# rasmusbarr/nudge

Hardware: AMD Instinct MI355X
Metric: simulation steps/s (contacts solved/s alongside), 1M-box drop scene (higher is better)
Workload: dtype f32

## Files before the change

### nudge_amd/csrc/nh_solve.hip

```cpp
#include "nh_internal.h"
#include <type_traits>
#include <atomic>
#include <string.h>
#include "nh_solver.h"
#include "nh_narrowphase.h"

__global__ __launch_bounds__(256) void k_gravity(const nh_DevState* __restrict__ st, const uint32_t* __restrict__ active, nh_BodyMomentum* __restrict__ momentum,
                                                 float gx_dt, float gy_dt, float gz_dt, float damping) {
	uint32_t n = st->active;
	for (uint32_t k = blockIdx.x * blockDim.x + threadIdx.x; k < n; k += gridDim.x * blockDim.x) {
		uint32_t i = active[k];
		nh_BodyMomentum m = momentum[i];
		nh_gravity_damping(m.velocity, m.angular_velocity, gx_dt, gy_dt, gz_dt, damping);
		momentum[i] = m;
	}
}

__global__ __launch_bounds__(256) void k_advance(const nh_DevState* __restrict__ st, const uint32_t* __restrict__ active, nh_Transform* __restrict__ xf,
                                                 const nh_BodyMomentum* __restrict__ momentum, uint8_t* __restrict__ idle, float time_step) {
	uint32_t n = st->active;
	for (uint32_t k = blockIdx.x * blockDim.x + threadIdx.x; k < n; k += gridDim.x * blockDim.x) {
		uint32_t i = active[k];
		nh_Transform t = xf[i];
		nh_BodyMomentum m = momentum[i];
// ... 309 lines not shown
			for (int q = 0; q < M; ++q) cid[q] = (uint32_t)q < cnt ? adj[b + q] : 0u;
#pragma unroll
			for (int q = 0; q < M; ++q) {
				miss[q] = false; wx[q] = wy[q] = wz[q] = 0.0f;
				if ((uint32_t)q < cnt) {
					const uint32_t c = cid[q];
					is_a[q] = bodies[c].a == x;
					ctc[q] = contacts[c];
					if (FUSED) {
						const uint64_t t = cv.tags[c]; const uint32_t f = cv.features[c];
						const bool in = c < m;
						const uint64_t ct = in ? cv.ctags[c] : 0ull; const uint32_t cf = in ? cv.cfeatures[c] : 0u;
						nh_CachedContactImpulse wc = { { 0.0f, 0.0f, 0.0f }, 0.0f };
						if (in) wc = cv.cdata[c];
						const bool hit = in && ct == t && cf == f;
						if (hit) { wx[q] = wc.impulse[0]; wy[q] = wc.impulse[1]; wz[q] = wc.impulse[2]; }
						miss[q] = !hit;
					} else {
						float4 sv = states[c];
						s[q].normal = sv.x; s[q].friction_x = sv.y; s[q].friction_y = sv.z;
					}
				}
			}
			if (FUSED) {
#pragma unroll
				for (int q = 0; q < M; ++q) {
					if (miss[q]) {
						const uint32_t c = cid[q];
						const uint64_t t = cv.tags[c]; const uint32_t f = cv.features[c];
						uint32_t lo = 0, hi = m;
						while (lo < hi) { uint32_t mid = (lo + hi) >> 1; if (tag_less(cv.ctags[mid], cv.cfeatures[mid], t, f)) lo = mid + 1; else hi = mid; }
						if (lo < m && cv.ctags[lo] == t && cv.cfeatures[lo] == f) { nh_CachedContactImpulse w = cv.cdata[lo]; wx[q] = w.impulse[0]; wy[q] = w.impulse[1]; wz[q] = w.impulse[2]; }
					}
				}
			}
#pragma unroll
			for (int q = 0; q < M; ++q) {
				if ((uint32_t)q < cnt) {
					const nh_Contact& ct = ctc[q];
					nh_contact_in ci = { ct.position[0], ct.position[1], ct.position[2], ct.penetration, ct.normal[0], ct.normal[1], ct.normal[2], ct.friction };
					if (is_a[q]) nh_build_row(ci, posx, pos0, IX, I0, v.mass_inverse, z.mass_inverse, r[q]);
					else         nh_build_row(ci, pos0, posx, I0, IX, z.mass_inverse, v.mass_inverse, r[q]);
					if (FUSED) {
						if (is_a[q]) nh_warm_start(r[q], wx[q], wy[q], wz[q], v, z, s[q]);
						else         nh_warm_start(r[q], wx[q], wy[q], wz[q], z, v, s[q]);
					}
				}
			}
			for (uint32_t it = 0; it < iterations; ++it) {
#pragma unroll
				for (int q = 0; q < M; ++q) {
					if ((uint32_t)q < cnt) {
						if (is_a[q]) nh_apply_one(r[q], s[q], v, z); else nh_apply_one(r[q], s[q], z, v);
					}
				}
			}
#pragma unroll
			for (int q = 0; q < M; ++q)
				if ((uint32_t)q < cnt) {
					states[cid[q]] = make_float4(s[q].normal, s[q].friction_x, s[q].friction_y, 0.0f);
					nh_CachedContactImpulse o;
					nh_export_impulse(r[q], s[q], o.impulse[0], o.impulse[1], o.impulse[2]);
					o.unused = 0.0f;
					impulses[cid[q]] = o;
				}
		} else {
			const nh_inertia IXn = body_inertia(xf, props, x);
			const nh_Transform txn = xf[x];
			const nh_f3 posxn = nh_make3(txn.position[0], txn.position[1], txn.position[2]);
			for (uint32_t it = 0; it < iterations; ++it) {
				for (uint32_t q = b; q < e; ++q) {
					uint32_t c = adj[q];
					const bool x_is_a = bodies[c].a == x;
					nh_Contact ct = contacts[c];
					nh_contact_in ci = { ct.position[0], ct.position[1], ct.position[2], ct.penetration, ct.normal[0], ct.normal[1], ct.normal[2], ct.friction };
					nh_row r;
					if (x_is_a) nh_build_row(ci, posxn, pos0, IXn, I0, v.mass_inverse, z.mass_inverse, r);
					else        nh_build_row(ci, pos0, posxn, I0, IXn, z.mass_inverse, v.mass_inverse, r);
					float4 sv = states[c];
					nh_state s = { sv.x, sv.y, sv.z };
					if (x_is_a) nh_apply_one(r, s, v, z); else nh_apply_one(r, s, z, v);
					states[c] = make_float4(s.normal, s.friction_x, s.friction_y, 0.0f);
					if (it + 1 == iterations) {
						nh_CachedContactImpulse o;
						nh_export_impulse(r, s, o.impulse[0], o.impulse[1], o.impulse[2]);
						o.unused = 0.0f;
						impulses[c] = o;
					}
				}
			}
		}
		store_vel(momentum, x, v);
	}
}

#define NH_HINT_NONE 0xFFFFFFFFu

__device__ __forceinline__ bool cache_probe(const nh_CacheView& cv, uint32_t m, uint32_t guess, uint64_t t, uint32_t f, float& wx, float& wy, float& wz) {
	if (guess < m) {
		const uint64_t ct = cv.ctags[guess];
		const uint32_t cf = cv.cfeatures[guess];
		const float4 w = *reinterpret_cast<const float4*>(cv.cdata + guess);
		if (ct == t && cf == f) { wx = w.x; wy = w.y; wz = w.z; return true; }
	}
	return false;
}

__device__ __noinline__ float4 cache_search(const uint64_t* __restrict__ ctags, const uint32_t* __restrict__ cfeatures, const nh_CachedContactImpulse* __restrict__ cdata,
                                            uint32_t m, uint32_t guess, uint64_t t, uint32_t f) {
	const float4 none = make_float4(0.0f, 0.0f, 0.0f, 0.0f);
	uint32_t lo = 0, hi = m;
	if (guess != NH_HINT_NONE && m) {
		const uint32_t g = guess < m ? guess : m - 1;
		const uint32_t w0 = g >= 4 ? g - 4 : 0, w1 = g + 4 < m ? g + 4 : m;
		bool below = false, above = false;
		for (uint32_t k = w0; k < w1; ++k) {
			const uint64_t ct = ctags[k]; const uint32_t cf = cfeatures[k];
			if (ct == t && cf == f) return *reinterpret_cast<const float4*>(cdata + k);
			if (tag_less(ct, cf, t, f)) below = true; else above = true;
		}
		if ((below || w0 == 0) && (above || w1 == m)) return none;
		if (!below) hi = w0; else lo = w1;
	}
	while (lo < hi) { uint32_t mid = (lo + hi) >> 1; if (tag_less(ctags[mid], cfeatures[mid], t, f)) lo = mid + 1; else hi = mid; }
	if (lo < m && ctags[lo] == t && cfeatures[lo] == f) return *reinterpret_cast<const float4*>(cdata + lo);
	return none;
}

struct nh_ob_slot { float4 c0, c1, w; };

#ifndef NH_SOLVER_WPE
#define NH_SOLVER_WPE 2
#endif
struct nh_StillView { const uint32_t* body_rec; const uint32_t* body_pos; const uint32_t* cnt_sorted; uint32_t* start_sorted; const uint32_t* raw_feature; uint32_t* sc_feat; uint32_t* sc_count; uint32_t pair_cap;
                     const int2* delta; uint32_t parity; };

template<int MAXC, bool FUSED, bool CONTIG = false, int NW = 4, bool STILL = false, bool AHEAD = false, bool PAIR = false, bool PART = false>
__global__ __launch_bounds__(64 * NW) __attribute__((amdgpu_waves_per_eu(MAXC == 4 ? NH_SOLVER_WPE : 1, MAXC == 4 ? NH_SOLVER_WPE : 1))) void k_solve_one_body(uint32_t nbodies, const uint8_t* __restrict__ body_class, const uint32_t* __restrict__ off, const uint32_t* __restrict__ adj,
                                                        const nh_BodyPair* __restrict__ bodies, const nh_BodyProperties* __restrict__ props, nh_BodyMomentum* __restrict__ momentum,
                                                        float4* __restrict__ states, uint32_t iterations,
                                                        const nh_Contact* __restrict__ contacts, nh_Transform* xf, nh_CachedContactImpulse* __restrict__ impulses,
                                                        nh_CacheView cv, uint32_t* __restrict__ hint, uint32_t cls_a, uint32_t cls_b, uint32_t require_inert,
                                                        const uint2* __restrict__ simple = nullptr, nh_FusedStep fs = nh_FusedStep(), nh_StillView sv = nh_StillView(),
                                                        nh_AheadView av = nh_AheadView()) {
	constexpr int M = MAXC;
	const bool keep_states = !(require_inert & 2u);
	if (nbodies == 0u) return;
	if (STILL && CONTIG && NW == 1 && !PART && (fs.bits & 8u) && blockIdx.x != 0u) {
		const uint32_t x0 = blockIdx.x * 64u + threadIdx.x;
		const uint32_t i0 = (x0 < nbodies) ? (uint32_t)fs.idle[x0] : 0xffu;
		if (__builtin_amdgcn_ballot_w64(i0 != 0xffu) == 0ull) return;
	}
	uint32_t inert_word = (require_inert & 1u) ? cv.st->static_inert : 1u;
	if (STILL) {
		const nh_BodyMomentum m0 = momentum[0];
		const nh_BodyProperties p0 = props[0];
		const bool inert = nh_is_inert(m0.velocity, m0.angular_velocity, p0.inertia_inverse, p0.mass_inverse);
		if (!inert && blockIdx.x == 0 && threadIdx.x == 0) atomicMax(&const_cast<nh_DevState*>(cv.st)->still_failed_seq, fs.seq);
		if (!inert || cv.st->still_failed_seq >= fs.guard_seq) {
			if (fs.host_counters && blockIdx.x == 0 && threadIdx.x == 0 && !(PART && fs.part == 1u)) {
				const volatile uint32_t* src = reinterpret_cast<const volatile uint32_t*>(cv.st);
#pragma unroll
				for (uint32_t k = 0; k < NH_COUNTER_WORDS; ++k) fs.host_counters[k] = src[k];
				__threadfence_system();
				__hip_atomic_store(fs.host_counters + NH_COUNTER_WORDS, fs.seq, __ATOMIC_RELEASE, __HIP_MEMORY_SCOPE_SYSTEM);
			}
			return;
		}
		inert_word = 1u;
	}
	__shared__ nh_ob_slot s_slot[NW][64 * M];
	__shared__ uint32_t s_cid[NW][64 * M];
	__shared__ uint32_t s_hint[NW][64], s_first[NW][64];
	__shared__ int2 s_delta[STILL ? NH_DELTA_MAX : 1];
	__shared__ uint32_t s_col[AHEAD ? NW : 1][AHEAD ? 64 : 1];
	__shared__ uint32_t s_pk[PAIR ? NW : 1][PAIR ? 4 : 1][PAIR ? 64 : 1];
	uint32_t n_delta = 0;
	if (STILL) {
		n_delta = cv.st->delta_overflow[sv.parity] ? 0u : min(cv.st->delta_count[sv.parity], NH_DELTA_MAX);
		for (uint32_t k = threadIdx.x; k < n_delta; k += blockDim.x) s_delta[k] = sv.delta[sv.parity * NH_DELTA_MAX + k];
		if (blockIdx.x == 0 && threadIdx.x == 0 && !(PART && fs.part == 1u)) {
			const uint32_t nrec = cv.st->records;
			int shift = 0;
			for (uint32_t k = 0; k < n_delta; ++k) shift += sv.delta[sv.parity * NH_DELTA_MAX + k].y;
			const uint32_t total = sv.start_sorted[nrec] + (uint32_t)shift;
			if (shift) sv.start_sorted[nrec] = total;
			nh_DevState* const stw = const_cast<nh_DevState*>(cv.st);
			stw->contacts = total;
			uint32_t n_sleeping = stw->still_sleeping[sv.parity], n_culled = stw->still_culled[sv.parity];
			if (fs.bits & 4u) {
				for (uint32_t k = 0; k < NH_SLEEP_PARTS; ++k) { n_sleeping += stw->sleep_part[sv.parity][k][0]; n_culled += stw->sleep_part[sv.parity][k][1]; }
			}
			stw->active = (nbodies - 1u) - min(stw->still_asleep[sv.parity], nbodies - 1u); stw->sleeping = n_sleeping; stw->culled = n_culled;
			if (fs.host_counters) {
				const volatile uint32_t* src = reinterpret_cast<const volatile uint32_t*>(cv.st);
#pragma unroll
				for (uint32_t k = 0; k < NH_COUNTER_WORDS; ++k) fs.host_counters[k] = src[k];
				__threadfence_system();
				__hip_atomic_store(fs.host_counters + NH_COUNTER_WORDS, fs.seq, __ATOMIC_RELEASE, __HIP_MEMORY_SCOPE_SYSTEM);
			}
		}
		__syncthreads();
	}
	if (!STILL && fs.host_counters && blockIdx.x == 0 && threadIdx.x == 0) {
		const volatile uint32_t* src = reinterpret_cast<const volatile uint32_t*>(cv.st);
#pragma unroll
		for (uint32_t k = 0; k < NH_COUNTER_WORDS; ++k) fs.host_counters[k] = src[k];
		__threadfence_system();
		__hip_atomic_store(fs.host_counters + NH_COUNTER_WORDS, fs.seq, __ATOMIC_RELEASE, __HIP_MEMORY_SCOPE_SYSTEM);
	}
	const uint32_t wave = threadIdx.x >> 6, lane = nh_lane();
	nh_ob_slot* slot = s_slot[wave];
	uint32_t* scid = s_cid[wave];
	const uint32_t m = (FUSED && !STILL) ? cv.st->cache : 0u;
	nh_CachedContactImpulse* const out_impulses = STILL ? const_cast<nh_CachedContactImpulse*>(cv.cdata) : impulses;
	const uint32_t rounded = (nbodies + (64u * NW - 1u)) / (64u * NW) * (64u * NW);
	uint32_t x = blockIdx.x * blockDim.x + threadIdx.x;
	if (PART && fs.part == 1u) {
		const uint32_t cnt_listed = *fs.xcount;
		x = x < cnt_listed ? fs.xlist[x] : 0u;
	}
	else if (x >= rounded) return;
	do {
		const uint32_t xc = min(x, nbodies - 1u);
		const uint32_t my_class = STILL ? 0u : body_class[xc];
		uint2 sp = make_uint2(0u, 0u);
		uint32_t h = NH_HINT_NONE;
		if (CONTIG && !STILL) sp = simple[xc];
		if (FUSED && !STILL) h = hint[xc];
		uint32_t br = NH_BODY_REC_NONE, bpos = 0u, idle0 = 0u;
		if (STILL) { br = sv.body_rec[xc]; bpos = sv.body_pos[xc]; if (CONTIG && (fs.bits & 4u)) idle0 = fs.idle[xc]; }
		uint32_t col = 0xFFFFFFFFu;
		if (AHEAD) col = av.body_col[xc];
		if (!inert_word) return;
		bool mine = STILL ? (x >= 1u && x < nbodies && idle0 != 0xffu) : (x < nbodies && (my_class == cls_a || my_class == cls_b));
		if (PART && fs.part == 2u && fs.xskip[xc] != 0u) mine = false;
		const uint32_t wave_x0 = x - lane;
		uint32_t b = 0, cnt = 0;
		if (!STILL && __builtin_amdgcn_ballot_w64(mine) == 0ull) { if (CONTIG) break; x += gridDim.x * blockDim.x; continue; }
		if (STILL && CONTIG && (fs.bits & 8u) && __builtin_amdgcn_ballot_w64(mine) == 0ull) break;
		if (!mine) { sp = make_uint2(0u, 0u); h = NH_HINT_NONE; br = NH_BODY_REC_NONE; }
		uint32_t cid[M];
		uint32_t first = 0xFFFFFFFFu;
		uint32_t still_base = 0, still_rec = 0;
		bool still_has = false;
		uint32_t st_start = 0, st_cnt = 0, st_oc = 0;
		uint32_t nf[M], of[M];
		uint32_t sl[M], jm[M];
#pragma unroll
		for (int k = 0; k < M; ++k) { nf[k] = 0u; of[k] = 0u; sl[k] = (uint32_t)k; jm[k] = 0xFFFFFFFFu; }
		if (STILL) {
			still_has = br != NH_BODY_REC_NONE;
			still_rec = still_has ? (br & ~NH_BODY_REC_IS_A) : 0u;
			const uint32_t n_bb = min(cv.st->pairs, sv.pair_cap);
			still_base = still_rec < n_bb ? 4u * still_rec : 4u * n_bb + (still_rec - n_bb);
			const uint32_t bp = still_has ? bpos : 0u;
			st_cnt = sv.cnt_sorted[bp]; st_start = sv.start_sorted[bp]; st_oc = sv.sc_count[still_rec];
			if (PAIR) {
				const uint2 kp = still_rec < n_bb ? av.kept[still_rec] : av.kept[av.kept_cap - 1u - (still_rec - n_bb)];
				const uint64_t pk = av.rec_key[still_rec];
				s_pk[wave][0][lane] = kp.x; s_pk[wave][1][lane] = kp.y; s_pk[wave][2][lane] = (uint32_t)pk; s_pk[wave][3][lane] = (uint32_t)(pk >> 32);
			}
#pragma unroll
			for (int k = 0; k < M; ++k) { nf[k] = sv.raw_feature[still_base + k]; of[k] = sv.sc_feat[still_base + k]; }
			s_first[wave][lane] = still_has ? still_base : 0xFFFFFFFFu;
		} else {
		if (CONTIG) cnt = sp.y & 15u;
		else if (mine) { b = off[x]; cnt = off[x + 1] - b; }
#pragma unroll
		for (int q = 0; q < M; ++q) {
			if (CONTIG) cid[q] = (uint32_t)q < cnt ? sp.x + ((sp.y >> (4 + 3 * q)) & 7u) : 0xFFFFFFFFu;
			else cid[q] = (uint32_t)q < cnt ? adj[b + q] : 0xFFFFFFFFu;
			first = min(first, cid[q]);
		}
		}
		if (!STILL) {
#pragma unroll
			for (int q = 0; q < M; ++q) scid[lane * M + q] = cid[q];
			s_hint[wave][lane] = h; s_first[wave][lane] = first;
		}
		const bool ghost_lane = AHEAD && fs.ghost_first != 0u && x >= fs.ghost_first;
		if (AHEAD) { if (!mine || ghost_lane) col = 0xFFFFFFFFu; s_col[wave][lane] = col; }
		__builtin_amdgcn_wave_barrier();
		uint32_t sc[M], sflags[M];
		float4 sc0[M], sc1[M], sw[M];
		uint64_t stag[M], sctag[M];
		uint32_t sfeat[M], scfeat[M], sguess[M];
#pragma unroll
		for (int k = 0; k < M; ++k) {
			const uint32_t e = 64u * k + lane, j = e / M;
			if (STILL) { const uint32_t bj = s_first[wave][j]; sc[k] = bj != 0xFFFFFFFFu ? bj + (e - j * M) : 0xFFFFFFFFu; }
			else sc[k] = scid[e];
			const uint32_t c = sc[k] != 0xFFFFFFFFu ? sc[k] : 0u;
			sc0[k] = reinterpret_cast<const float4*>(contacts + c)[0];
			sc1[k] = reinterpret_cast<const float4*>(contacts + c)[1];
			sflags[k] = (!CONTIG && bodies[c].a == wave_x0 + j) ? 2u : 0u;
			if (STILL) {
				sw[k] = *reinterpret_cast<const float4*>(cv.cdata + c);
			} else if (FUSED) {
				const uint32_t hj = s_hint[wave][j];
				sguess[k] = hj != NH_HINT_NONE ? hj + (sc[k] - s_first[wave][j]) : sc[k];
				const uint32_t g = sguess[k] < m ? sguess[k] : 0u;
				stag[k] = cv.tags[c]; sfeat[k] = cv.features[c];
				sctag[k] = cv.ctags[g]; scfeat[k] = cv.cfeatures[g];
				sw[k] = *reinterpret_cast<const float4*>(cv.cdata + g);
			} else {
				sw[k] = states[c];
			}
		}
		float4 m0 = make_float4(0, 0, 0, 0), m1 = m0, pr = m0, t0 = m0, t1 = make_float4(0, 0, 0, 1);
		uint32_t idle_early = 0;
		if (mine) {
			m0 = reinterpret_cast<const float4*>(momentum + x)[0]; m1 = reinterpret_cast<const float4*>(momentum + x)[1];
			pr = *reinterpret_cast<const float4*>(props + x);
			t0 = reinterpret_cast<const float4*>(xf + x)[0]; t1 = reinterpret_cast<const float4*>(xf + x)[1];
			if (CONTIG && (fs.bits & 2u)) idle_early = (STILL && (fs.bits & 4u)) ? idle0 : fs.idle[x];
			if (CONTIG && (fs.bits & 1u)) {
				float vel[3] = { m0.x, m0.y, m0.z }, ang[3] = { m1.x, m1.y, m1.z };
				nh_gravity_damping(vel, ang, fs.gx_dt, fs.gy_dt, fs.gz_dt, fs.damping);
				m0.x = vel[0]; m0.y = vel[1]; m0.z = vel[2]; m1.x = ang[0]; m1.y = ang[1]; m1.z = ang[2];
			}
		}
#pragma unroll
		for (int k = 0; k < M; ++k) {
			const uint32_t e = 64u * k + lane;
			nh_ob_slot o;
			o.c0 = make_float4(0, 0, 0, 0); o.c1 = o.c0; o.w = o.c0;
			if (sc[k] != 0xFFFFFFFFu) {
				uint32_t flags = sflags[k];
				o.c0 = sc0[k]; o.c1 = sc1[k];
				if (STILL) {
					o.w = make_float4(sw[k].x, sw[k].y, sw[k].z, __uint_as_float(flags));
				} else if (FUSED) {
					const bool hit = sguess[k] < m && sctag[k] == stag[k] && scfeat[k] == sfeat[k];
					if (!hit) flags |= 1u;
					o.w = hit ? make_float4(sw[k].x, sw[k].y, sw[k].z, __uint_as_float(flags)) : make_float4(0.0f, 0.0f, 0.0f, __uint_as_float(flags));
				} else {
					o.w = make_float4(sw[k].x, sw[k].y, sw[k].z, __uint_as_float(flags));
				}
			}
			slot[e] = o;
		}
		if (STILL) {
			uint32_t oc = 0;
			if (still_has) {
				cnt = min(st_cnt, 4u); oc = min(st_oc, 4u);
				uint32_t start = st_start;
				int shift = 0;
				for (uint32_t k = 0; k < n_delta; ++k) shift += (uint32_t)s_delta[k].x < bpos ? s_delta[k].y : 0;
				if (shift) { start += (uint32_t)shift; sv.start_sorted[bpos] = start; }
				st_start = start;
			}
			uint32_t ci[M], key[M];
#pragma unroll
			for (int k = 0; k < M; ++k) {
				uint32_t r = 0;
#pragma unroll
				for (int j = 0; j < M; ++j) r += ((uint32_t)j < cnt && (uint32_t)k < cnt && (nf[j] < nf[k] || (nf[j] == nf[k] && j < k))) ? 1u : 0u;
				const bool on = (uint32_t)k < cnt;
				ci[k] = on ? st_start + r : 0xFFFFFFFFu;
				key[k] = on ? slot_key_of(ci[k], nullptr) : 0xFFFFFFFFu;
				sl[k] = (uint32_t)k;
			}
#pragma unroll
			for (int q = 1; q < M; ++q) {
#pragma unroll
				for (int j = q; j > 0; --j) {
					const bool sw2 = (key[j] < key[j - 1]) || (key[j] == key[j - 1] && ci[j] < ci[j - 1]);
					const uint32_t tc = sw2 ? ci[j - 1] : ci[j], tk = sw2 ? key[j - 1] : key[j], ts = sw2 ? sl[j - 1] : sl[j];
					ci[j - 1] = sw2 ? ci[j] : ci[j - 1]; key[j - 1] = sw2 ? key[j] : key[j - 1]; sl[j - 1] = sw2 ? sl[j] : sl[j - 1];
					ci[j] = tc; key[j] = tk; sl[j] = ts;
				}
			}
#pragma unroll
			for (int q = 0; q < M; ++q) {
				const bool on = (uint32_t)q < cnt;
				uint32_t f = 0, wj = 0xFFFFFFFFu;
#pragma unroll
				for (int k = 0; k < M; ++k) if (sl[q] == (uint32_t)k) f = nf[k];
#pragma unroll
				for (int j = M - 1; j >= 0; --j) if ((uint32_t)j < oc && of[j] == f) wj = (uint32_t)j;
				jm[q] = on ? wj : 0xFFFFFFFFu;
				cid[q] = on ? still_base + sl[q] : 0xFFFFFFFFu;
				scid[lane * M + q] = cid[q];
			}
			if (still_has) {
#pragma unroll
				for (int k = 0; k < M; ++k) if ((uint32_t)k < cnt) sv.sc_feat[still_base + k] = nf[k];
				sv.sc_count[still_rec] = cnt;
			}
		}
		__builtin_amdgcn_wave_barrier();
		nh_vel v = { m0.x, m0.y, m0.z, pr.w, m1.x, m1.y, m1.z, m1.w };
		const nh_quat qx = { t1.x, t1.y, t1.z, t1.w };
		const nh_inertia IX = nh_world_inertia(qx, pr.x, pr.y, pr.z);
		const nh_f3 posx = nh_make3(t0.x, t0.y, t0.z);
		nh_row1 r[M];
		nh_state s[M];
		bool is_a[M];
		nh_div_deferred dd;
		const nh_vel v0 = v;
		nh_state w0[M];
#pragma unroll
		for (int q = 0; q < M; ++q) {
			is_a[q] = false;
			w0[q].normal = 0.0f; w0[q].friction_x = 0.0f; w0[q].friction_y = 0.0f;
			if ((uint32_t)q < cnt) {
				const nh_ob_slot o = slot[lane * M + (STILL ? sl[q] : (uint32_t)q)];
				const uint32_t flags = STILL ? 0u : __float_as_uint(o.w.w);
				is_a[q] = STILL ? (br & NH_BODY_REC_IS_A) != 0 : (CONTIG ? ((sp.y >> 28) & 1u) != 0 : (flags & 2u) != 0);
				nh_contact_in ci = { o.c0.x, o.c0.y, o.c0.z, o.c0.w, o.c1.x, o.c1.y, o.c1.z, o.c1.w };
				nh_build_row1(ci, posx, IX, v.mass_inverse, is_a[q], r[q]);
				if (FUSED) {
					float wx = o.w.x, wy = o.w.y, wz = o.w.z;
					if (STILL) {
						const float4 wv = slot[lane * M + (jm[q] != 0xFFFFFFFFu ? jm[q] : 0u)].w;
						const bool hit = jm[q] != 0xFFFFFFFFu;
						wx = hit ? wv.x : 0.0f; wy = hit ? wv.y : 0.0f; wz = hit ? wv.z : 0.0f;
					}
					if (!STILL && (flags & 1u)) {
						const float4 found = cache_search(cv.ctags, cv.cfeatures, cv.cdata, m, h != NH_HINT_NONE ? h + (cid[q] - first) : cid[q], cv.tags[cid[q]], cv.features[cid[q]]);
						wx = found.x; wy = found.y; wz = found.z;
					}
					w0[q].normal = wx; w0[q].friction_x = wy; w0[q].friction_y = wz;
					nh_warm_start1(r[q], wx, wy, wz, v, is_a[q], s[q], dd);
				} else {
					w0[q].normal = o.w.x; w0[q].friction_x = o.w.y; w0[q].friction_y = o.w.z;
					s[q] = w0[q];
				}
			}
		}
		if (FUSED && !STILL && mine) hint[x] = first;
		nh_xform pp_x = nh_xform();
		float4 pp_min = make_float4(0, 0, 0, 0), pp_max = pp_min, pp_shape = pp_min;
		uint32_t pp_tag = 0, pp_own_tag = 0, pp_partner = 0xFFFFFFFFu, pp_bits = 0;
		if (PAIR && CONTIG && (fs.bits & 2u) && mine && still_has && s_col[wave][lane] != 0xFFFFFFFFu) {
			const uint32_t ah_col = s_col[wave][lane];
			const uint32_t kx = s_pk[wave][0][lane], ky = s_pk[wave][1][lane];
			const uint32_t index_mask = av.gen ? NH_GEN_INDEX : 0xFFFFFFFFu;
			const uint32_t ca = kx & index_mask, cb = ky & index_mask;
			pp_partner = ca == ah_col ? cb : ca;
			pp_bits = 1u | ((ca != ah_col && cb != ah_col) ? 4u : 0u);
			if (av.gen && cv.st->moved_count != 0u && !((uint32_t)(av.gen[ca] & 0x7Fu) == (kx >> NH_GEN_SHIFT) && (uint32_t)(av.gen[cb] & 0x7Fu) == (ky >> NH_GEN_SHIFT))) pp_bits |= 2u;
			pp_x = av.xf[pp_partner]; pp_min = av.aabb_min[pp_partner]; pp_max = av.aabb_max[pp_partner];
			if (pp_partner < av.nbox) pp_shape = *reinterpret_cast<const float4*>(av.box_data + pp_partner);
			else pp_shape.x = av.sph_data[pp_partner - av.nbox].radius;
			pp_tag = av.ctag[pp_partner]; pp_own_tag = av.ctag[ah_col];
		}
		float4* const s_ah = reinterpret_cast<float4*>(slot);
		float ah_rad = 0.0f;
		if (AHEAD) {
			__builtin_amdgcn_wave_barrier();
			const uint32_t c0 = s_col[wave][lane];
			const uint32_t cc = c0 != 0xFFFFFFFFu ? c0 : 0u;
			const bool is_box = cc < av.nbox;
			const float4* lp = reinterpret_cast<const float4*>(is_box ? av.box_xf + cc : av.sph_xf + (cc - av.nbox));
			const float4* sp4 = is_box ? reinterpret_cast<const float4*>(av.box_data + cc) : lp;
			if (!is_box) ah_rad = av.sph_data[cc - av.nbox].radius;
			nh_glds16(lp, &s_ah[lane]); nh_glds16(lp + 1, &s_ah[64u + lane]);
			nh_glds16(av.fat_box + 2u * (size_t)cc, &s_ah[128u + lane]); nh_glds16(av.fat_box + 2u * (size_t)cc + 1u, &s_ah[192u + lane]);
			nh_glds16(sp4, &s_ah[256u + lane]);
		}
		const bool none_a = CONTIG && __builtin_amdgcn_ballot_w64(mine && (STILL ? (still_has && (br & NH_BODY_REC_IS_A) != 0) : ((sp.y >> 28) & 1u) != 0)) == 0;
		auto sweeps = [&](auto& div) {
			if (none_a) {
				for (uint32_t it = 0; it < iterations; ++it) {
#pragma unroll
					for (int q = 0; q < M; ++q)
						if ((uint32_t)q < cnt) nh_apply_one1(r[q], s[q], v, false, div);
				}
			} else {
				for (uint32_t it = 0; it < iterations; ++it) {
#pragma unroll
					for (int q = 0; q < M; ++q)
						if ((uint32_t)q < cnt) nh_apply_one1(r[q], s[q], v, is_a[q], div);
				}
			}
		};
		sweeps(dd);
		if (__builtin_expect(dd.bad != 0ull, 0)) {
			nh_div_exact ex;
			v = v0;
#pragma unroll
			for (int q = 0; q < M; ++q) {
				if ((uint32_t)q < cnt) {
					if (FUSED) nh_warm_start1(r[q], w0[q].normal, w0[q].friction_x, w0[q].friction_y, v, is_a[q], s[q], ex);
					else s[q] = w0[q];
				}
			}
			sweeps(ex);
		}
		float4 a0 = make_float4(0, 0, 0, 0), a1 = a0;
		uint32_t idle_in = 0;
		const bool advance_here = CONTIG && (fs.bits & 2u) && mine;
		float4 ah_l0 = make_float4(0, 0, 0, 0), ah_l1 = ah_l0, ah_fmn = ah_l0, ah_fmx = ah_l0, ah_sz = ah_l0;
		uint32_t ah_col = 0xFFFFFFFFu;
		if (AHEAD) {
			ah_col = s_col[wave][lane];
			asm volatile("s_waitcnt vmcnt(0)" ::: "memory");
			ah_l0 = s_ah[lane]; ah_l1 = s_ah[64u + lane]; ah_fmn = s_ah[128u + lane]; ah_fmx = s_ah[192u + lane]; ah_sz = s_ah[256u + lane];
		}
		if (advance_here) { a0 = t0; a1 = t1; idle_in = idle_early; }
		__builtin_amdgcn_wave_barrier();
#pragma unroll
		for (int q = 0; q < M; ++q) {
			if ((uint32_t)q < cnt) {
				float ox, oy, oz;
				nh_export_impulse1(r[q], s[q], ox, oy, oz);
				slot[lane * M + q].c0 = make_float4(s[q].normal, s[q].friction_x, s[q].friction_y, 0.0f);
				slot[lane * M + q].c1 = make_float4(ox, oy, oz, 0.0f);
			}
		}
		__builtin_amdgcn_wave_barrier();
#pragma unroll
		for (int k = 0; k < M; ++k) {
			const uint32_t e = 64u * k + lane;
			const uint32_t c = scid[e];
			if (c != 0xFFFFFFFFu) {
				if (keep_states) states[c] = slot[e].c0;
				*reinterpret_cast<float4*>(out_impulses + c) = slot[e].c1;
			}
		}
		if (mine) {
			reinterpret_cast<float4*>(momentum + x)[0] = make_float4(v.vx, v.vy, v.vz, v.mass_inverse);
			reinterpret_cast<float4*>(momentum + x)[1] = make_float4(v.wx, v.wy, v.wz, v.w_unused);
		}
		uint32_t nmin[3] = { 0xffffffffu, 0xffffffffu, 0xffffffffu }, nmax[3] = { 0u, 0u, 0u }, ntop = 0u;
		bool nfail = false;
		int pp_count = 0;
		float pair_scale = 0.0f;
		if (PAIR) {
			__builtin_amdgcn_wave_barrier();
#pragma unroll
			for (int k = 0; k < M; ++k) scid[lane * M + k] = 0xFFFFFFFFu;
			const nh_DevState* const sp = cv.st;
			const nh_f3 smin = nh_make3(nh_float_unflip(sp->still_smin[sv.parity][0]), nh_float_unflip(sp->still_smin[sv.parity][1]), nh_float_unflip(sp->still_smin[sv.parity][2]));
			const nh_f3 smax = nh_make3(nh_float_unflip(sp->still_smax[sv.parity][0]), nh_float_unflip(sp->still_smax[sv.parity][1]), nh_float_unflip(sp->still_smax[sv.parity][2]));
			pair_scale = nh_morton_scale(smin, smax);
			if (sp->pair_unowned > av.unowned_cap) nfail = true;
		}
		if (advance_here) {
			float pos[3] = { a0.x, a0.y, a0.z }, rot[4] = { a1.x, a1.y, a1.z, a1.w };
			const float vel[3] = { v.vx, v.vy, v.vz }, ang[3] = { v.wx, v.wy, v.wz };
			const uint8_t idle_out = nh_advance_body(pos, rot, vel, ang, (uint8_t)idle_in, fs.time_step);
			fs.idle[x] = idle_out;
			reinterpret_cast<float4*>(xf + x)[0] = make_float4(pos[0], pos[1], pos[2], a0.w);
			reinterpret_cast<float4*>(xf + x)[1] = make_float4(rot[0], rot[1], rot[2], rot[3]);
			if (AHEAD && !ghost_lane) {
				ntop = idle_out; nfail = idle_out == 0xffu;
				const uint32_t c = ah_col;
				if (c != 0xFFFFFFFFu) {
					const bool is_box = c < av.nbox;
					const float4 l0 = ah_l0, l1 = ah_l1, fmn = ah_fmn, fmx = ah_fmx;
					float4 sz = ah_sz;
					if (!is_box) sz.x = ah_rad;
					const nh_quat bq = { rot[0], rot[1], rot[2], rot[3] };
					const nh_quat lq = { l1.x, l1.y, l1.z, l1.w };
					const nh_f3 p = nh_rotate(bq, nh_make3(l0.x, l0.y, l0.z)) + nh_make3(pos[0], pos[1], pos[2]);
					const nh_quat q = nh_qmul(bq, lq);
					float sx, sy, sz2;
					if (is_box) {
						const nh_m33 m = nh_matrix(q);
						const nh_f3 c0 = m.c0 * sz.x, c1 = m.c1 * sz.y, c2 = m.c2 * sz.z;
						sx = fabsf(c0.x) + fabsf(c1.x) + fabsf(c2.x);
						sy = fabsf(c0.y) + fabsf(c1.y) + fabsf(c2.y);
						sz2 = fabsf(c0.z) + fabsf(c1.z) + fabsf(c2.z);
					} else {
						sx = sy = sz2 = sz.x;
					}
					const float mnx = p.x - sx, mny = p.y - sy, mnz = p.z - sz2, mxx = p.x + sx, mxy = p.y + sy, mxz = p.z + sz2;
					float4* const wx = reinterpret_cast<float4*>(av.xf) + 2u * (size_t)c;
					wx[0] = make_float4(p.x, p.y, p.z, l0.w);
					wx[1] = make_float4(q.x, q.y, q.z, q.s);
					av.aabb_min[c] = make_float4(mnx, mny, mnz, l0.w);
					av.aabb_max[c] = make_float4(mxx, mxy, mxz, __uint_as_float(0u));
					nfail |= !(mnx >= fmn.x && mny >= fmn.y && mnz >= fmn.z && mxx <= fmx.x && mxy <= fmx.y && mxz <= fmx.z);
					nmin[0] = nmax[0] = nh_float_flip(mnx); nmin[1] = nmax[1] = nh_float_flip(mny); nmin[2] = nmax[2] = nh_float_flip(mnz);
					if (PAIR && (pp_bits & 1u)) {
						const float4 omin = make_float4(mnx, mny, mnz, l0.w), omax = make_float4(mxx, mxy, mxz, 0.0f);
						nh_xform OX; OX.px = p.x; OX.py = p.y; OX.pz = p.z; OX.body = __float_as_uint(l0.w); OX.qx = q.x; OX.qy = q.y; OX.qz = q.z; OX.qs = q.s;
						const bool hit = nh_aabb_overlap(omin, omax, pp_min, pp_max) && __float_as_uint(pp_min.w) != OX.body && !(pp_bits & 2u);
						const float ddx = mnx - pp_min.x, ddy = mny - pp_min.y, ddz = mnz - pp_min.z;
						const float far = 2.0f;
						const bool partner_first = ddx >= 0.0f && ddy >= 0.0f && ddz >= 0.0f && fmaxf(fmaxf(ddx, ddy), ddz) * pair_scale >= far;
						const bool own_first = ddx <= 0.0f && ddy <= 0.0f && ddz <= 0.0f && fmaxf(fmaxf(-ddx, -ddy), -ddz) * pair_scale >= far;
						bool pfail = (pp_bits & 4u) != 0u || (hit && !partner_first && !own_first) || __float_as_uint(pp_min.w) != 0u;
						if (pfail) atomicAdd(&const_cast<nh_DevState*>(cv.st)->pair_diag[(hit && !partner_first && !own_first) ? 0 : 1], 1u);
						uint64_t key = ~0ull;
						uint32_t body_a = 0, body_b = 0;
						nh_bb_result bb;
						bb.kind = 0; bb.mask = 0;
						nh_contact_out single;
						single.px = single.py = single.pz = single.penetration = single.nx = single.ny = single.nz = 0.0f; single.friction = 0.5f; single.feature = 0u;
						if (hit && !pfail) {
							const bool a_is_own = partner_first;
							const nh_xform A = a_is_own ? OX : pp_x, B = a_is_own ? pp_x : OX;
							const uint32_t ta = a_is_own ? pp_own_tag : pp_tag, tb = a_is_own ? pp_tag : pp_own_tag;
							const bool own_sph = !is_box, par_sph = pp_partner >= av.nbox;
							const bool a_sph = a_is_own ? own_sph : par_sph, b_sph = a_is_own ? par_sph : own_sph;
							const float own_size[3] = { sz.x, sz.y, sz.z }, par_size[3] = { pp_shape.x, pp_shape.y, pp_shape.z };
							const float ra = a_is_own ? sz.x : pp_shape.x, rb = a_is_own ? pp_shape.x : sz.x;
							if (!a_sph && !b_sph) {
								nh_box_box_eval(A, B, a_is_own ? own_size : par_size, a_is_own ? par_size : own_size, ta, tb, bb);
								pp_count = nh_bb_count(bb);
								key = (uint64_t)(bb.swapped ? tb : ta) | ((uint64_t)(bb.swapped ? ta : tb) << 32);
								body_a = bb.swapped ? B.body : A.body; body_b = bb.swapped ? A.body : B.body;
							} else if (a_sph && b_sph) {
								pp_count = nh_sphere_sphere(rb, ra, B, A, &single);
								key = (uint64_t)tb | ((uint64_t)ta << 32);
								body_a = B.body; body_b = A.body;
							} else {
								const nh_xform BX = a_sph ? B : A, SP = a_sph ? A : B;
								const bool box_is_own = a_sph ? !a_is_own : a_is_own;
								pp_count = nh_box_sphere(box_is_own ? own_size : par_size, a_sph ? ra : rb, BX, SP, &single);
								key = (uint64_t)(a_sph ? tb : ta) | ((uint64_t)(a_sph ? ta : tb) << 32);
								body_a = BX.body; body_b = SP.body;
							}
						}
						{
							const uint64_t was_key = (uint64_t)s_pk[wave][2][lane] | ((uint64_t)s_pk[wave][3][lane] << 32);
							const bool vanished = !hit;
							const bool same_key = was_key == key || vanished;
							bool ok = same_key && pp_count <= 4;
							if (ok && pp_count) ok = (body_a == 0u) != (body_b == 0u);
							if (!ok) { pfail = true; pp_count = 0; bb.kind = 0; atomicAdd(&const_cast<nh_DevState*>(cv.st)->pair_diag[1], 1u); }
						}
						nfail |= pfail;
						if (pp_count) {
							nh_ob_slot* const stage = slot + lane * M;
							if (bb.kind == 2) {
								int k = 0;
#pragma unroll
								for (int index = 0; index < 16; ++index) {
									if (((bb.mask >> index) & 1u) && k < pp_count && k < M) {
										nh_contact_out o;
										nh_bb_contact(bb, index, bb.fx[index], bb.fy[index], bb.fz[index], bb.penetration[index], bb.tags[index], o);
										stage[k].c0 = make_float4(o.px, o.py, o.pz, o.penetration); stage[k].c1 = make_float4(o.nx, o.ny, o.nz, o.friction); stage[k].w.x = __uint_as_float(o.feature);
										scid[lane * M + k] = still_base + (uint32_t)k;
										++k;
									}
								}
							} else {
								const nh_contact_out o = bb.kind == 1 ? bb.edge : single;
								stage[0].c0 = make_float4(o.px, o.py, o.pz, o.penetration); stage[0].c1 = make_float4(o.nx, o.ny, o.nz, o.friction); stage[0].w.x = __uint_as_float(o.feature);
								scid[lane * M] = still_base;
							}
						}
						av.rec[still_rec].count = (uint32_t)pp_count;
						if (st_cnt != (uint32_t)pp_count) {
							nh_DevState* const stw = const_cast<nh_DevState*>(cv.st);
							const uint32_t np2 = sv.parity ^ 1u;
							av.cnt_sorted[bpos] = (uint32_t)pp_count;
							if (!stw->delta_overflow[np2]) {
								const uint32_t k = atomicAdd(&stw->delta_count[np2], 1u);
								if (k < NH_DELTA_MAX) av.delta[np2 * NH_DELTA_MAX + k] = make_int2((int)bpos, pp_count - (int)st_cnt);
								else { stw->delta_overflow[np2] = 1u; if (!av.delta_scan) nfail = true; }
							}
						}
					}
				}
			}
		}
		if (PAIR) {
			__builtin_amdgcn_wave_barrier();
#pragma unroll
			for (int k = 0; k < M; ++k) {
				const uint32_t e = 64u * k + lane;
				const uint32_t c = scid[e];
				if (c != 0xFFFFFFFFu) {
					float4* dp = reinterpret_cast<float4*>(av.raw_data + c);
					dp[0] = slot[e].c0; dp[1] = slot[e].c1;
					av.raw_feature[c] = __float_as_uint(slot[e].w.x);
				}
			}
		}
		if (AHEAD) {
			nh_DevState* const stw = const_cast<nh_DevState*>(cv.st);
			const uint32_t np = sv.parity ^ 1u;
#pragma unroll
			for (int k = 0; k < 3; ++k) {
				for (int d = 32; d >= 1; d >>= 1) { nmin[k] = min(nmin[k], (uint32_t)__shfl_xor((int)nmin[k], d)); nmax[k] = max(nmax[k], (uint32_t)__shfl_xor((int)nmax[k], d)); }
			}
			for (int d = 32; d >= 1; d >>= 1) ntop = max(ntop, (uint32_t)__shfl_xor((int)ntop, d));
			const unsigned long long bad = __ballot(nfail);
			uint32_t* const part = &stw->ahead_part[np][(blockIdx.x * NW + wave) & (NH_AHEAD_PARTS - 1u)][0];
			const uint32_t mine_min = lane == 0u ? nmin[0] : (lane == 1u ? nmin[1] : nmin[2]);
			const uint32_t mine_max = lane == 3u ? nmax[0] : (lane == 4u ? nmax[1] : (lane == 5u ? nmax[2] : ntop));
			if (lane < 3u) atomicMin(&part[lane], mine_min);
			else if (lane < 7u) atomicMax(&part[lane], mine_max);
			else if (lane == 7u && bad != 0ull) atomicMax(&stw->ahead_failed_seq, fs.seq + 1u);
		}
		__builtin_amdgcn_wave_barrier();
// ... 1313 lines not shown
```

Measured before the change: 3936.

## Hoist device-state and per-body loads ahead of inert check in still solver

In the STILL path of the one-body solver, the device-state counters (failed seq, pairs, records, delta count/overflow, moved, unowned, smin/smax) and the per-lane body words (record, position, idle, column, momentum, properties, transform) are now loaded at kernel entry. Empty asm constraints force those loads to be issued early, so their latency overlaps the inert check and setup instead of stalling later. The first delta entry is prefetched per thread, and the pair-key LDS stores are deferred. This raises register pressure and issues loads even for blocks that exit early, and it reads momentum and xf before any write ordering the old code relied on.

After: 4085, median of 6. 3.8% higher.

```diff
diff --git a/nudge_amd/csrc/nh_solve.hip b/nudge_amd/csrc/nh_solve.hip
--- a/nudge_amd/csrc/nh_solve.hip
+++ b/nudge_amd/csrc/nh_solve.hip
@@ -485,12 +485,39 @@
 		if (__builtin_amdgcn_ballot_w64(i0 != 0xffu) == 0ull) return;
 	}
 	uint32_t inert_word = (require_inert & 1u) ? cv.st->static_inert : 1u;
+	uint32_t x = blockIdx.x * blockDim.x + threadIdx.x;
+	const bool lane_early = STILL && !(PART && fs.part == 1u);
+	uint32_t h_failed = 0u, h_pairs = 0u, h_records = 0u, h_dcount = 0u, h_dover = 0u, h_moved = 0u, h_unowned = 0u;
+	uint32_t h_smin[3] = { 0u, 0u, 0u }, h_smax[3] = { 0u, 0u, 0u };
+	int2 h_delta = make_int2(0, 0);
+	uint32_t l_br = NH_BODY_REC_NONE, l_bpos = 0u, l_idle = 0u, l_col = 0xFFFFFFFFu;
+	float4 l_m0 = make_float4(0, 0, 0, 0), l_m1 = l_m0, l_pr = l_m0, l_t0 = l_m0, l_t1 = l_m0;
+	auto lane_words = [&](uint32_t xi) {
+		l_br = sv.body_rec[xi]; l_bpos = sv.body_pos[xi];
+		if (CONTIG && (fs.bits & 6u)) l_idle = fs.idle[xi];
+		if (AHEAD) l_col = av.body_col[xi];
+		l_m0 = reinterpret_cast<const float4*>(momentum + xi)[0]; l_m1 = reinterpret_cast<const float4*>(momentum + xi)[1];
+		l_pr = *reinterpret_cast<const float4*>(props + xi);
+		l_t0 = reinterpret_cast<const float4*>(xf + xi)[0]; l_t1 = reinterpret_cast<const float4*>(xf + xi)[1];
+	};
+	float pair_scale0 = 0.0f;
 	if (STILL) {
+		const nh_DevState* const st0 = cv.st;
 		const nh_BodyMomentum m0 = momentum[0];
 		const nh_BodyProperties p0 = props[0];
+		h_failed = st0->still_failed_seq; h_pairs = st0->pairs; h_records = st0->records;
+		h_dcount = st0->delta_count[sv.parity]; h_dover = st0->delta_overflow[sv.parity];
+		if (PAIR) {
+			h_moved = st0->moved_count; h_unowned = st0->pair_unowned;
+			for (int k = 0; k < 3; ++k) { h_smin[k] = st0->still_smin[sv.parity][k]; h_smax[k] = st0->still_smax[sv.parity][k]; }
+		}
+		h_delta = sv.delta[sv.parity * NH_DELTA_MAX + (threadIdx.x & (NH_DELTA_MAX - 1u))];
+		if (lane_early) lane_words(min(x, nbodies - 1u));
+		asm volatile("" :: "s"(h_failed), "s"(h_pairs), "s"(h_records), "s"(h_dcount), "s"(h_dover), "v"(h_delta.x), "v"(h_delta.y), "v"(l_br), "v"(l_bpos), "v"(l_idle), "v"(l_col) : "memory");
+		if (PAIR) asm volatile("" :: "s"(h_moved), "s"(h_unowned), "s"(h_smin[0]), "s"(h_smin[1]), "s"(h_smin[2]), "s"(h_smax[0]), "s"(h_smax[1]), "s"(h_smax[2]));
 		const bool inert = nh_is_inert(m0.velocity, m0.angular_velocity, p0.inertia_inverse, p0.mass_inverse);
 		if (!inert && blockIdx.x == 0 && threadIdx.x == 0) atomicMax(&const_cast<nh_DevState*>(cv.st)->still_failed_seq, fs.seq);
-		if (!inert || cv.st->still_failed_seq >= fs.guard_seq) {
+		if (!inert || h_failed >= fs.guard_seq) {
 			if (fs.host_counters && blockIdx.x == 0 && threadIdx.x == 0 && !(PART && fs.part == 1u)) {
 				const volatile uint32_t* src = reinterpret_cast<const volatile uint32_t*>(cv.st);
 #pragma unroll
@@ -501,6 +528,8 @@
 			return;
 		}
 		inert_word = 1u;
+		if (PAIR) pair_scale0 = nh_morton_scale(nh_make3(nh_float_unflip(h_smin[0]), nh_float_unflip(h_smin[1]), nh_float_unflip(h_smin[2])),
+		                                        nh_make3(nh_float_unflip(h_smax[0]), nh_float_unflip(h_smax[1]), nh_float_unflip(h_smax[2])));
 	}
 	__shared__ nh_ob_slot s_slot[NW][64 * M];
 	__shared__ uint32_t s_cid[NW][64 * M];
@@ -510,10 +539,11 @@
 	__shared__ uint32_t s_pk[PAIR ? NW : 1][PAIR ? 4 : 1][PAIR ? 64 : 1];
 	uint32_t n_delta = 0;
 	if (STILL) {
-		n_delta = cv.st->delta_overflow[sv.parity] ? 0u : min(cv.st->delta_count[sv.parity], NH_DELTA_MAX);
-		for (uint32_t k = threadIdx.x; k < n_delta; k += blockDim.x) s_delta[k] = sv.delta[sv.parity * NH_DELTA_MAX + k];
+		n_delta = h_dover ? 0u : min(h_dcount, NH_DELTA_MAX);
+		if (threadIdx.x < n_delta) s_delta[threadIdx.x] = h_delta;
+		for (uint32_t k = threadIdx.x + blockDim.x; k < n_delta; k += blockDim.x) s_delta[k] = sv.delta[sv.parity * NH_DELTA_MAX + k];
 		if (blockIdx.x == 0 && threadIdx.x == 0 && !(PART && fs.part == 1u)) {
-			const uint32_t nrec = cv.st->records;
+			const uint32_t nrec = h_records;
 			int shift = 0;
 			for (uint32_t k = 0; k < n_delta; ++k) shift += sv.delta[sv.parity * NH_DELTA_MAX + k].y;
 			const uint32_t total = sv.start_sorted[nrec] + (uint32_t)shift;
@@ -548,7 +578,6 @@
 	const uint32_t m = (FUSED && !STILL) ? cv.st->cache : 0u;
 	nh_CachedContactImpulse* const out_impulses = STILL ? const_cast<nh_CachedContactImpulse*>(cv.cdata) : impulses;
 	const uint32_t rounded = (nbodies + (64u * NW - 1u)) / (64u * NW) * (64u * NW);
-	uint32_t x = blockIdx.x * blockDim.x + threadIdx.x;
 	if (PART && fs.part == 1u) {
 		const uint32_t cnt_listed = *fs.xcount;
 		x = x < cnt_listed ? fs.xlist[x] : 0u;
@@ -562,9 +591,9 @@
 		if (CONTIG && !STILL) sp = simple[xc];
 		if (FUSED && !STILL) h = hint[xc];
 		uint32_t br = NH_BODY_REC_NONE, bpos = 0u, idle0 = 0u;
-		if (STILL) { br = sv.body_rec[xc]; bpos = sv.body_pos[xc]; if (CONTIG && (fs.bits & 4u)) idle0 = fs.idle[xc]; }
+		if (STILL) { if (!lane_early) lane_words(xc); br = l_br; bpos = l_bpos; if (CONTIG && (fs.bits & 4u)) idle0 = l_idle; }
 		uint32_t col = 0xFFFFFFFFu;
-		if (AHEAD) col = av.body_col[xc];
+		if (AHEAD) col = STILL ? l_col : av.body_col[xc];
 		if (!inert_word) return;
 		bool mine = STILL ? (x >= 1u && x < nbodies && idle0 != 0xffu) : (x < nbodies && (my_class == cls_a || my_class == cls_b));
 		if (PART && fs.part == 2u && fs.xskip[xc] != 0u) mine = false;
@@ -578,6 +607,8 @@
 		uint32_t still_base = 0, still_rec = 0;
 		bool still_has = false;
 		uint32_t st_start = 0, st_cnt = 0, st_oc = 0;
+		uint2 st_kp = make_uint2(0u, 0u);
+		uint64_t st_pk = 0ull;
 		uint32_t nf[M], of[M];
 		uint32_t sl[M], jm[M];
 #pragma unroll
@@ -585,18 +616,17 @@
 		if (STILL) {
 			still_has = br != NH_BODY_REC_NONE;
 			still_rec = still_has ? (br & ~NH_BODY_REC_IS_A) : 0u;
-			const uint32_t n_bb = min(cv.st->pairs, sv.pair_cap);
+			const uint32_t n_bb = min(h_pairs, sv.pair_cap);
 			still_base = still_rec < n_bb ? 4u * still_rec : 4u * n_bb + (still_rec - n_bb);
 			const uint32_t bp = still_has ? bpos : 0u;
 			st_cnt = sv.cnt_sorted[bp]; st_start = sv.start_sorted[bp]; st_oc = sv.sc_count[still_rec];
+			s_first[wave][lane] = still_has ? still_base : 0xFFFFFFFFu;
 			if (PAIR) {
-				const uint2 kp = still_rec < n_bb ? av.kept[still_rec] : av.kept[av.kept_cap - 1u - (still_rec - n_bb)];
-				const uint64_t pk = av.rec_key[still_rec];
-				s_pk[wave][0][lane] = kp.x; s_pk[wave][1][lane] = kp.y; s_pk[wave][2][lane] = (uint32_t)pk; s_pk[wave][3][lane] = (uint32_t)(pk >> 32);
+				st_kp = still_rec < n_bb ? av.kept[still_rec] : av.kept[av.kept_cap - 1u - (still_rec - n_bb)];
+				st_pk = av.rec_key[still_rec];
 			}
 #pragma unroll
 			for (int k = 0; k < M; ++k) { nf[k] = sv.raw_feature[still_base + k]; of[k] = sv.sc_feat[still_base + k]; }
-			s_first[wave][lane] = still_has ? still_base : 0xFFFFFFFFu;
 		} else {
 		if (CONTIG) cnt = sp.y & 15u;
 		else if (mine) { b = off[x]; cnt = off[x + 1] - b; }
@@ -643,11 +673,19 @@
 		}
 		float4 m0 = make_float4(0, 0, 0, 0), m1 = m0, pr = m0, t0 = m0, t1 = make_float4(0, 0, 0, 1);
 		uint32_t idle_early = 0;
+		if (STILL) {
+			asm volatile("" ::: "memory");
+			if (PAIR) { s_pk[wave][0][lane] = st_kp.x; s_pk[wave][1][lane] = st_kp.y; s_pk[wave][2][lane] = (uint32_t)st_pk; s_pk[wave][3][lane] = (uint32_t)(st_pk >> 32); }
+		}
 		if (mine) {
+			if (STILL) {
+				m0 = l_m0; m1 = l_m1; pr = l_pr; t0 = l_t0; t1 = l_t1;
+			} else {
 			m0 = reinterpret_cast<const float4*>(momentum + x)[0]; m1 = reinterpret_cast<const float4*>(momentum + x)[1];
 			pr = *reinterpret_cast<const float4*>(props + x);
 			t0 = reinterpret_cast<const float4*>(xf + x)[0]; t1 = reinterpret_cast<const float4*>(xf + x)[1];
-			if (CONTIG && (fs.bits & 2u)) idle_early = (STILL && (fs.bits & 4u)) ? idle0 : fs.idle[x];
+			}
+			if (CONTIG && (fs.bits & 2u)) idle_early = STILL ? l_idle : fs.idle[x];
 			if (CONTIG && (fs.bits & 1u)) {
 				float vel[3] = { m0.x, m0.y, m0.z }, ang[3] = { m1.x, m1.y, m1.z };
 				nh_gravity_damping(vel, ang, fs.gx_dt, fs.gy_dt, fs.gz_dt, fs.damping);
@@ -774,7 +812,7 @@
 			const uint32_t ca = kx & index_mask, cb = ky & index_mask;
 			pp_partner = ca == ah_col ? cb : ca;
 			pp_bits = 1u | ((ca != ah_col && cb != ah_col) ? 4u : 0u);
-			if (av.gen && cv.st->moved_count != 0u && !((uint32_t)(av.gen[ca] & 0x7Fu) == (kx >> NH_GEN_SHIFT) && (uint32_t)(av.gen[cb] & 0x7Fu) == (ky >> NH_GEN_SHIFT))) pp_bits |= 2u;
+			if (av.gen && h_moved != 0u && !((uint32_t)(av.gen[ca] & 0x7Fu) == (kx >> NH_GEN_SHIFT) && (uint32_t)(av.gen[cb] & 0x7Fu) == (ky >> NH_GEN_SHIFT))) pp_bits |= 2u;
 			pp_x = av.xf[pp_partner]; pp_min = av.aabb_min[pp_partner]; pp_max = av.aabb_max[pp_partner];
 			if (pp_partner < av.nbox) pp_shape = *reinterpret_cast<const float4*>(av.box_data + pp_partner);
 			else pp_shape.x = av.sph_data[pp_partner - av.nbox].radius;
@@ -866,11 +904,8 @@
 			__builtin_amdgcn_wave_barrier();
 #pragma unroll
 			for (int k = 0; k < M; ++k) scid[lane * M + k] = 0xFFFFFFFFu;
-			const nh_DevState* const sp = cv.st;
-			const nh_f3 smin = nh_make3(nh_float_unflip(sp->still_smin[sv.parity][0]), nh_float_unflip(sp->still_smin[sv.parity][1]), nh_float_unflip(sp->still_smin[sv.parity][2]));
-			const nh_f3 smax = nh_make3(nh_float_unflip(sp->still_smax[sv.parity][0]), nh_float_unflip(sp->still_smax[sv.parity][1]), nh_float_unflip(sp->still_smax[sv.parity][2]));
-			pair_scale = nh_morton_scale(smin, smax);
-			if (sp->pair_unowned > av.unowned_cap) nfail = true;
+			pair_scale = pair_scale0;
+			if (h_unowned > av.unowned_cap) nfail = true;
 		}
 		if (advance_here) {
 			float pos[3] = { a0.x, a0.y, a0.z }, rot[4] = { a1.x, a1.y, a1.z, a1.w };
```
